# CognitiveAISystems/pogema

Measured on AMD Instinct MI355X. Metric: agent-steps/sec (whole node), 64-agent 64x64 grid, batch=8192 envs, higher is better.
Workload: dtype u32

## Files before the change

include/pogema_amd.h:

```cpp
#ifndef POGEMA_AMD_H
#define POGEMA_AMD_H

#include <stddef.h>
#include <stdint.h>

#ifdef __cplusplus
extern "C" {
#endif

#define PGX_ABI_VERSION 6

#define PGX_OK 0
#define PGX_E_INVALID (-1)
#define PGX_E_HIP (-2)
#define PGX_E_NOMEM (-3)
#define PGX_E_STATE (-4)
#define PGX_E_PLACEMENT (-5)

#define PGX_COLLISION_PRIORITY 0
#define PGX_COLLISION_BLOCK_BOTH 1
#define PGX_COLLISION_SOFT 2

#define PGX_ON_TARGET_FINISH 0
#define PGX_ON_TARGET_RESTART 1
// ... 49 lines not shown
typedef struct pgx_env pgx_env;

int pgx_abi_version(void);
const char* pgx_last_error(void);

int pgx_create(const pgx_config* cfg, int device, pgx_env** out);
int pgx_destroy(pgx_env* env);
int pgx_check_config(const pgx_config* cfg);

int64_t pgx_obs_elems(const pgx_env* env);
int64_t pgx_agent_elems(const pgx_env* env);

int pgx_reset_from_state(pgx_env* env, const uint8_t* obstacles, const int32_t* agent_xy,
                         const int32_t* target_xy, void* stream);

int pgx_reset_random(pgx_env* env, float density, uint64_t seed, const uint8_t* shared_map,
                     const uint8_t* env_mask, int32_t max_retries, void* stream);

int pgx_regenerate(pgx_env* env, const uint8_t* env_mask, float density, uint64_t seed, const uint8_t* shared_map,
                   int32_t max_retries, void* obs, void* stream);
int64_t pgx_regenerate_failures(pgx_env* env, void* stream);

int pgx_set_map_pool(pgx_env* env, const uint8_t* maps, int32_t num_maps, int32_t* capacity_out, void* stream);
int pgx_reset_pool(pgx_env* env, uint64_t seed, const uint8_t* env_mask, int32_t max_retries, void* stream);
int pgx_regenerate_pool(pgx_env* env, const uint8_t* env_mask, uint64_t seed, int32_t max_retries, void* obs,
                        void* stream);
int pgx_get_map_index(pgx_env* env, int32_t* map_index, void* stream);

int pgx_get_map(pgx_env* env, uint8_t* obstacles, void* stream);

int pgx_step(pgx_env* env, const void* actions, int action_dtype, void* obs, float* rewards,
             uint8_t* terminated, uint8_t* truncated, uint8_t* is_active, void* stream);

int pgx_step_held(pgx_env* env, const void* actions, int action_dtype, void* obs, uint8_t* held, int32_t refresh,
                  float* rewards, uint8_t* terminated, uint8_t* truncated, uint8_t* is_active, void* stream);
int pgx_held_available(const pgx_env* env);

int pgx_xcd_shares(pgx_env* env, int32_t* shares);
int pgx_xcd_tune(pgx_env* env, void* obs, void* obs_alt, int32_t rounds, float* us_equal, float* us_tuned, void* stream);

typedef struct pgx_geometry {
    int32_t lanes_per_env;
    int32_t waves;
    int32_t envs_per_wave;
    int32_t multi_wave;
    int32_t p16;
    int32_t stagger;
    int32_t store_policy;
    int32_t state_stores;
    int32_t grid;
    int32_t lds_bytes;
    int32_t for_rollout;
    int32_t xcd_aware;
} pgx_geometry;
int pgx_get_geometry(const pgx_env* env, int32_t for_rollout, pgx_geometry* out);

typedef struct pgx_rollout_io {
    const void* actions;
    void* obs;
    float* rewards;
    uint8_t* terminated;
    uint8_t* truncated;
    uint8_t* is_active;
    uint8_t* episode_done;
    float* metrics;
    int32_t action_dtype;
    int32_t obs_slots;
    int64_t obs_slot_stride;
    uint64_t policy_seed;
// ... 140 lines not shown
```

pogema_amd/_lib.py:

```python
from __future__ import annotations

import ctypes as C
import os

_HERE = os.path.dirname(os.path.abspath(__file__))
LIB_PATH = os.environ.get("PGX_LIB") or os.path.join(_HERE, "libpogema_amd.so")

PGX_ABI_VERSION = 6

COLLISION_SYSTEMS = {"priority": 0, "block_both": 1, "soft": 2}
ON_TARGET = {"finish": 0, "restart": 1, "nothing": 2}
ACTION_DTYPES = {"int8": 0, "int32": 1, "int64": 2}
SOFT_VERTEX_RULES = {"lowest_index": 0, "all_stay": 1}
SOFT_OCCUPANCY = {"index_order": 0, "exact": 1}
COOP_REWARDS = {"all_solved": 0, "per_agent": 1}
BAD_ACTIONS = {"noop": 0, "flag": 1}
LIFELONG_RNGS = {"build": 0, "numpy": 1}
def _obs_dtypes():
    import torch
    return {torch.float32: 0, torch.uint8: 1, torch.bfloat16: 2, torch.float16: 3}


def obs_elem_bytes(dtype) -> int:
    import torch
# ... 9 lines not shown
    def __contains__(self, k):
        self._fill()
        return dict.__contains__(self, k)

    def __getitem__(self, k):
        self._fill()
        return dict.__getitem__(self, k)


OBS_DTYPES = _LazyObsDtypes()
METRIC_NAMES = ("ISR", "CSR", "ep_length", "SoC", "makespan", "avg_throughput")
MAX_OBS_RADIUS, MAX_AGENTS, MAX_SIDE = 15, 1024, 1024
MAX_NEIGHBOURS = 32
DIRECTIONS_FORMATS = {"float32": 0, "uint8": 1, "bits": 2}
SHIELD_TIE_BREAKS = {None: 0, "distance": 1}
MAX_PLAN_HORIZON = 256
PLAN_FIXED_PRIORITY = 1
OUTCOMES = ("STAY", "MOVED", "OBSTACLE", "SWAP", "OCCUPIED", "FOLLOW", "CONTESTED")
NUM_OUTCOMES = len(OUTCOMES)
POLICY_CHANNELS = {"obstacles": 0, "agents": 1, "target": 2, "other_goals": 3, "up": 4, "down": 5, "left": 6, "right": 7}
NUM_CHANNELS = len(POLICY_CHANNELS)
COPY_NO_CACHE = 1
DEFAULT_POLICY_CHANNELS = ("obstacles", "agents", "target", "up", "down", "left", "right")
GLOBAL_CHANNELS = {"obstacles": 0, "agents": 1, "targets": 2, "agent_ids": 3, "target_ids": 4}
NUM_GLOBAL_CHANNELS = len(GLOBAL_CHANNELS)
DEFAULT_GLOBAL_CHANNELS = ("obstacles", "agents", "targets")
GLOBAL_ID_CHANNELS = ("agent_ids", "target_ids")
GLOBAL_ID_MAX = {1: 255, 2: 256}
GLOBAL_BAND_CELLS = 8192


EXPORTED_SYMBOLS = (
    "pgx_abi_version", "pgx_last_error", "pgx_create", "pgx_check_config", "pgx_destroy", "pgx_obs_elems", "pgx_agent_elems",
    "pgx_reset_from_state", "pgx_reset_random", "pgx_regenerate", "pgx_regenerate_failures", "pgx_get_map", "pgx_step", "pgx_step_held", "pgx_held_available", "pgx_observe", "pgx_set_metrics_buffers", "pgx_get_state", "pgx_generate", "pgx_place_agents",
    "pgx_snapshot_bytes", "pgx_save_snapshot", "pgx_load_snapshot", "pgx_time_observe", "pgx_bad_action_count",
    "pgx_buffers_create", "pgx_buffers_ptr", "pgx_buffers_get_info", "pgx_buffers_destroy", "pgx_set_targets",
    "pgx_np_streams", "pgx_np_streams_host", "pgx_np_generate", "pgx_np_generate_host", "pgx_rollout", "pgx_buffers_stride", "pgx_buffers_drop", "pgx_xcd_shares", "pgx_xcd_tune", "pgx_buffers_create_at", "pgx_time_observe_pair", "pgx_buffers_va_reserved", "pgx_get_geometry",
    "pgx_expert_actions", "pgx_set_map_pool", "pgx_reset_pool", "pgx_regenerate_pool", "pgx_get_map_index",
    "pgx_cost_to_go", "pgx_cost_to_go_bytes", "pgx_cost_to_go_builds", "pgx_visible_agents", "pgx_pibt_actions",
    "pgx_goal_directions", "pgx_shield_actions", "pgx_pibt_plan", "pgx_move_outcomes",
    "pgx_policy_input", "pgx_copy_envs", "pgx_global_state", "pgx_global_state_check",
)


class PgxError(RuntimeError):
    def __init__(self, code: int, message: str):
        super().__init__(f"pogema_amd engine error {code}: {message}")
        self.code = code


class PgxBuffersInfo(C.Structure):
    _fields_ = [("bytes", C.c_int64), ("count", C.c_int32), ("spread", C.c_int32), ("candidates", C.c_int32),
                ("reserved0", C.c_int32), ("same_zone_us", C.c_float), ("final_us", C.c_float), ("spacer_gib", C.c_double),
                ("buffer_gbs", C.c_float), ("reserved1", C.c_float)]


class PgxGeometry(C.Structure):
    _fields_ = [(n, C.c_int32) for n in ("lanes_per_env", "waves", "envs_per_wave", "multi_wave", "p16", "stagger",
                                          "store_policy", "state_stores", "grid", "lds_bytes", "for_rollout", "xcd_aware")]


class PgxRolloutIO(C.Structure):
    _fields_ = [("actions", C.c_void_p), ("obs", C.c_void_p), ("rewards", C.c_void_p), ("terminated", C.c_void_p),
                ("truncated", C.c_void_p), ("is_active", C.c_void_p), ("episode_done", C.c_void_p), ("metrics", C.c_void_p),
                ("action_dtype", C.c_int32), ("obs_slots", C.c_int32), ("obs_slot_stride", C.c_int64),
                ("policy_seed", C.c_uint64), ("policy_step0", C.c_int64), ("actions_out", C.c_void_p)]

# ... 96 lines not shown
    lib.pgx_move_outcomes.restype = C.c_int
    lib.pgx_policy_input.argtypes = [vp, C.POINTER(i32), i32, i32, vp, vp]
    lib.pgx_policy_input.restype = C.c_int
    lib.pgx_global_state.argtypes = [vp, C.POINTER(i32), i32, i32, vp, vp]
    lib.pgx_global_state.restype = C.c_int
    lib.pgx_global_state_check.argtypes = [i32, C.POINTER(i32), i32, i32, vp]
    lib.pgx_global_state_check.restype = C.c_int
    lib.pgx_copy_envs.argtypes = [vp, vp, vp, i32, i32, vp]
    lib.pgx_copy_envs.restype = C.c_int
    lib.pgx_set_map_pool.argtypes = [vp, vp, i32, vp, vp]
    lib.pgx_set_map_pool.restype = C.c_int
    lib.pgx_reset_pool.argtypes = [vp, u64, vp, i32, vp]
    lib.pgx_reset_pool.restype = C.c_int
    lib.pgx_regenerate_pool.argtypes = [vp, vp, u64, i32, vp, vp]
    lib.pgx_regenerate_pool.restype = C.c_int
    lib.pgx_get_map_index.argtypes = [vp, vp, vp]
    lib.pgx_get_map_index.restype = C.c_int
    lib.pgx_set_targets.argtypes = [vp, vp, vp, vp]
    lib.pgx_set_targets.restype = C.c_int
    lib.pgx_bad_action_count.argtypes = [vp, vp]
    lib.pgx_bad_action_count.restype = i64
    lib.pgx_time_observe.argtypes = [vp, vp, i32, C.POINTER(C.c_float), vp]
    lib.pgx_time_observe.restype = C.c_int
    lib.pgx_time_observe_pair.argtypes = [vp, vp, vp, i32, C.POINTER(C.c_float), vp]
    lib.pgx_time_observe_pair.restype = C.c_int
    lib.pgx_snapshot_bytes.argtypes = [vp]
    lib.pgx_snapshot_bytes.restype = i64
    lib.pgx_save_snapshot.argtypes = [vp, vp, vp]
    lib.pgx_load_snapshot.argtypes = [vp, vp, vp]
    lib.pgx_save_snapshot.restype = lib.pgx_load_snapshot.restype = C.c_int
    lib.pgx_step.argtypes = [vp, vp, C.c_int, vp, vp, vp, vp, vp, vp]
    lib.pgx_step_held.argtypes = [vp, vp, C.c_int, vp, vp, i32, vp, vp, vp, vp, vp]
    lib.pgx_held_available.argtypes = [vp]
    lib.pgx_step_held.restype = lib.pgx_held_available.restype = C.c_int
    lib.pgx_observe.argtypes = [vp, vp, vp]
    lib.pgx_set_metrics_buffers.argtypes = [vp, vp, vp]
    lib.pgx_get_state.argtypes = [vp, vp, vp, vp, vp, vp, vp]
    lib.pgx_generate.argtypes = [i32, i32, i32, i32, f32, u64, i64, i32, i32, vp, vp, vp]
    lib.pgx_place_agents.argtypes = [i32, i32, i32, i32, u64, i64, i32, i32, vp, i32, vp, vp]
    for name in ("pgx_create", "pgx_destroy", "pgx_reset_from_state", "pgx_reset_random", "pgx_regenerate", "pgx_get_map",
                 "pgx_step", "pgx_observe", "pgx_set_metrics_buffers", "pgx_set_metrics_buffers",
                 "pgx_get_state", "pgx_generate", "pgx_place_agents"):
        getattr(lib, name).restype = C.c_int
    if lib.pgx_abi_version() != PGX_ABI_VERSION:
        raise ImportError(f"{LIB_PATH}: ABI version {lib.pgx_abi_version()} != expected {PGX_ABI_VERSION}; rebuild")
    _lib = lib
    return lib


def check(status: int) -> None:
    if status != 0:
        msg = load().pgx_last_error()
        raise PgxError(status, msg.decode("utf-8", "replace") if msg else "unknown error")
```

pogema_amd/buffers.py:

```python
from __future__ import annotations

import atexit
import collections
import contextlib
import ctypes as C
import os
import threading

import numpy as np
import torch

from . import _lib

_TYPESTR = {torch.float32: "<f4", torch.uint8: "|u1", torch.float16: "<f2", torch.bfloat16: "<f2"}


class _Owner:

    def __init__(self, lib, handle):
        self._lib, self._handle = lib, handle

    def __del__(self):
        try:
            if self._handle is not None and self._handle.value:
# ... 284 lines not shown
            cdata = master.untyped_storage()._cdata
            base = hook(cdata)
            alias = master.detach()
            one = hook(cdata)
            view = alias[2:4].view(torch.int16)
            two = hook(cdata)
            del alias
            still = hook(cdata)
            del view
            back = hook(cdata)
            if not (one == base + 1 and two == base + 2 and still == base + 1 and back == base):
                why = f"torch._C._storage_Use_Count no longer counts tensors per storage ({base}, {one}, {two}, {still}, {back})"
        except Exception as exc:
            why = f"torch._C._storage_Use_Count self-test raised {exc!r}"
    if why is not None:
        import warnings
        warnings.warn(f"pogema_amd: {why} in torch {torch.__version__}; reuse_buffers='recycle' falls back to allocating "
                      f"fresh output tensors per step", RuntimeWarning, stacklevel=2)
        hook = None
    _HOOK = hook
    return hook


_UNSET = object()
_HOOK = _UNSET


class RecyclingOutputs:

    @staticmethod
    def available() -> bool:
        return storage_count_hook() is not None

    def __init__(self, obs_tensors, batch: int, agents: int, zone_ptrs=()):
        if not self.available():
            raise RuntimeError("torch._C._storage_Use_Count is missing or changed its meaning in this torch build")
        self._count = storage_count_hook()
        self._zone_ptrs = frozenset(int(p) for p in zone_ptrs)
        dev = obs_tensors[0].device
        n = batch * agents
        self._sets = []
        for obs in obs_tensors:
            block = torch.empty(n * 7 + 16, dtype=torch.uint8, device=dev)
            members = (obs, block[:4 * n].view(torch.float32).view(batch, agents),
                       block[4 * n:5 * n].view(torch.bool).view(batch, agents),
                       block[5 * n:6 * n].view(torch.bool).view(batch, agents),
                       block[6 * n:7 * n].view(torch.bool).view(batch, agents))
            storages = (obs.untyped_storage(), block.untyped_storage())
            self._sets.append((members, storages, tuple(st._cdata for st in storages)))
        del obs, block, members, storages
        self._idle = [tuple(self._count(c) for c in cdata) for _, _, cdata in self._sets]
        self._held = [torch.full((batch, agents), 255, dtype=torch.uint8, device=dev) for _ in self._sets]
        self._vouched = [None] * len(self._sets)
        self._next = 0
        self.taken = 0
        self.misses = 0

    def __len__(self):
        return len(self._sets)

    def obs_pointers(self):
        return [members[0].data_ptr() for members, _, _ in self._sets]

    def _is_idle(self, i: int) -> bool:
        cdata, idle = self._sets[i][2], self._idle[i]
        return self._count(cdata[0]) == idle[0] and self._count(cdata[1]) == idle[1]

    def free_sets(self) -> int:
        return sum(self._is_idle(i) for i in range(len(self._sets)))

    def retire(self):
        idle = [i for i in range(len(self._sets)) if self._is_idle(i)]
        out = [self._sets[i][0][0] for i in idle if self._sets[i][0][0].data_ptr() in self._zone_ptrs]
        for i in reversed(idle):
            del self._sets[i]
            del self._idle[i]
            del self._held[i]
            del self._vouched[i]
        self._next = 0
        return out

    def _take_index(self):
        n = len(self._sets)
        for k in range(n):
            i = (self._next + k) % n
            if self._is_idle(i):
                self._next = (i + 1) % n
                self.taken += 1
                return i
        self.misses += 1
        return None

    def _hand_out(self, i: int, with_obs: bool):
        m = self._sets[i][0]
        return (m[0].detach() if with_obs else None, m[1].detach(), m[2].detach(), m[3].detach(), m[4].detach())

    @staticmethod
    def _version(t):
        try:
            return t._version
        except Exception:
            return None

    def take(self, with_obs: bool = True):
        i = self._take_index()
        if i is None:
            return None
        if with_obs:
            self._vouched[i] = None
        return self._hand_out(i, with_obs)
# ... 15 lines not shown
```

pogema_amd/csrc/pgx_api.cpp:

```cpp
#include "../../include/pogema_amd.h"

#include <hip/hip_runtime.h>

#include <algorithm>
#include <cstdarg>
#include <cstdio>
#include <cstdlib>
#include <cstring>
#include <new>
#include <string>
#include <vector>

#include "pgx_internal.h"

namespace {
thread_local std::string g_err;
}

namespace pgx {
int fail_msg(int code, const char* fmt, ...) {
    char buf[512];
    va_list ap;
    va_start(ap, fmt);
    vsnprintf(buf, sizeof buf, fmt, ap);
// ... 881 lines not shown
int pgx_get_map(pgx_env* e, uint8_t* obstacles, void* stream) {
    if (!e || !obstacles) return fail_msg(PGX_E_INVALID, "pgx_get_map: null argument");
    DeviceGuard guard;
    if (const int rc = enter(guard, e, "pgx_get_map", true)) return rc;
    PGX_HIP(hipMemcpyAsync(obstacles, e->map_u8, (size_t)e->cfg.batch * e->cfg.height * e->cfg.width,
                           hipMemcpyDeviceToDevice, (hipStream_t)stream));
    return PGX_OK;
}

int pgx_step(pgx_env* e, const void* actions, int action_dtype, void* obs, float* rewards, uint8_t* terminated,
             uint8_t* truncated, uint8_t* is_active, void* stream) {
    if (!e || !actions || !rewards || !terminated || !truncated) return fail_msg(PGX_E_INVALID, "pgx_step: null argument");
    if (const int rc = check_action_dtype("pgx_step", action_dtype)) return rc;
    DeviceGuard guard;
    if (const int rc = enter(guard, e, "pgx_step", true)) return rc;
    pgx::StepParams p = step_params(e, e->geo);
    p.mode = pgx::MODE_STEP;
    p.action_dtype = action_dtype;
    p.actions = actions;
    p.obs = static_cast<float*>(obs);
    p.rewards = rewards;
    p.terminated = terminated;
    p.truncated = truncated;
    p.act_out = is_active;
    PGX_HIP(pgx::launch_step(p, e->geo, (hipStream_t)stream));
    return PGX_OK;
}

int pgx_held_available(const pgx_env* e) {
    if (!e) return 0;
    return pgx::held_available(e->geo, e->cfg.num_agents, e->W, obs_elem_bytes(e->cfg.obs_dtype)) ? 1 : 0;
}

int pgx_step_held(pgx_env* e, const void* actions, int action_dtype, void* obs, uint8_t* held, int32_t refresh, float* rewards,
                  uint8_t* terminated, uint8_t* truncated, uint8_t* is_active, void* stream) {
    if (!e || !obs || !held || !pgx_held_available(e))
        return pgx_step(e, actions, action_dtype, obs, rewards, terminated, truncated, is_active, stream);
    if (!actions || !rewards || !terminated || !truncated) return fail_msg(PGX_E_INVALID, "pgx_step_held: null argument");
    if (const int rc = check_action_dtype("pgx_step_held", action_dtype)) return rc;
    DeviceGuard guard;
    if (const int rc = enter(guard, e, "pgx_step_held", true)) return rc;
    pgx::StepParams p = step_params(e, e->geo);
    p.mode = pgx::MODE_STEP;
    p.action_dtype = action_dtype;
    p.actions = actions;
    p.obs = static_cast<float*>(obs);
    p.rewards = rewards;
    p.terminated = terminated;
    p.truncated = truncated;
    p.act_out = is_active;
    PGX_HIP(pgx::launch_step_held(p, e->geo, held, refresh != 0, (hipStream_t)stream));
    return PGX_OK;
}

int pgx_rollout(pgx_env* e, int32_t steps, const pgx_rollout_io* io, void* stream) {
    if (!e || !io || !io->rewards || !io->terminated || !io->truncated)
        return fail_msg(PGX_E_INVALID, "pgx_rollout: null argument");
    if (io->policy_step0 < 0 || io->policy_step0 > ((int64_t)1 << 40))
        return fail_msg(PGX_E_INVALID, "pgx_rollout: policy_step0 outside 0..2^40");
    if (steps < 1) return fail_msg(PGX_E_INVALID, "pgx_rollout: steps must be >= 1, got %d", steps);
    if (const int rc = check_action_dtype("pgx_rollout", io->action_dtype)) return rc;
    if (io->obs && io->obs_slots < 1) return fail_msg(PGX_E_INVALID, "pgx_rollout: obs given but obs_slots = %d", io->obs_slots);
    DeviceGuard guard;
    if (const int rc = enter(guard, e, "pgx_rollout", true)) return rc;
    pgx::StepParams p = step_params(e, e->geo_roll);
    p.mode = pgx::MODE_STEP;
    p.action_dtype = io->action_dtype;
    p.actions = io->actions;
    p.obs = static_cast<float*>(io->obs);
    p.rewards = io->rewards;
    p.terminated = io->terminated;
    p.truncated = io->truncated;
    p.act_out = io->is_active;
    p.metrics_out = io->metrics;
    p.episode_done = io->episode_done;
    const int64_t agents = (int64_t)e->cfg.batch * e->cfg.num_agents;
    const int64_t W = 2 * e->cfg.obs_radius + 1;
    static const int64_t action_bytes[3] = {1, 4, 8};
    pgx::RolloutParams rp;
    rp.steps = steps;
    rp.obs_slots = io->obs ? io->obs_slots : 1;
    rp.resident_bitmap = e->geo_roll.resident_bitmap ? 1 : 0;
    rp.reserved0 = 0;
    rp.actions_stride = agents * action_bytes[io->action_dtype];
// ... 554 lines not shown
```

pogema_amd/csrc/pgx_internal.h:

```cpp
#pragma once
#include <hip/hip_runtime.h>
#include <stddef.h>
#include <stdint.h>

namespace pgx {

int fail_msg(int code, const char* fmt, ...);

#define PGX_HIP(call)                                                                                                      \
    do {                                                                                                                   \
        const hipError_t e__ = (call);                                                                                     \
        if (e__ != hipSuccess)                                                                                             \
            return pgx::fail_msg(PGX_E_HIP, "%s failed: %s (%s:%d)", #call, hipGetErrorString(e__), __FILE__, __LINE__); \
    } while (0)

struct DeviceGuard {
    int prev = -1;
    bool changed = false;
    hipError_t err = hipSuccess;
    DeviceGuard() = default;
    explicit DeviceGuard(int dev) { (void)select(dev); }
    DeviceGuard(const DeviceGuard&) = delete;
    DeviceGuard& operator=(const DeviceGuard&) = delete;
    hipError_t select(int dev) {
// ... 78 lines not shown
    int32_t xcd_n[8];
    int32_t xcd_base[8];
    uint32_t flags;
    uint64_t seed;
    int64_t env_index_base;
    const uint32_t* obst;
    uint32_t* pos;
    uint32_t* tgt;
    uint8_t* active;
    int32_t* elapsed;
    const uint32_t* pos0;
    const uint32_t* tgt0;
    const uint32_t* comp_begin;
    const uint32_t* comp_len;
    const uint32_t* comp_cells;
    uint32_t* tcount;
    NpGen* np_state;
    const NpGen* np_state0;
    int4* macc;
    float* metrics_out;
    uint8_t* episode_done;
    uint32_t* bad_count;
    const void* actions;
    float* obs;
    float* rewards;
    uint8_t* terminated;
    uint8_t* truncated;
    uint8_t* act_out;
    const uint8_t* only;
    unsigned long long* dbg;
};

struct HeldParams {
    uint8_t* held;
    int32_t refresh;
    int32_t lds_word;
    int32_t words;
};

struct RolloutParams {
    int32_t steps;
    int32_t obs_slots;
    int32_t resident_bitmap;
    int32_t reserved0;
    int64_t actions_stride;
    int64_t agents_stride;
    int64_t envs_stride;
    int64_t obs_stride;
    uint64_t policy_seed;
    int64_t policy_step0;
    int8_t* actions_out;
};

struct StepGeometry {
    int G;
    int waves;
    int epw;
    bool multi_wave;
    bool p16;
    int stagger;
    int store_policy;
    int state_stores;
    bool big;
    bool pc;
    bool resident_bitmap;
    size_t lds_bytes;
    int grid;
    int32_t xcd_n[8], xcd_base[8];
};
StepGeometry step_geometry(int batch, int A, int bmw, int W, bool allow_p16, int epw_override, int obs_elem_bytes,
                           int waves_override, bool for_rollout = false);
hipError_t prepare_step(const StepGeometry& g, const StepGeometry& roll);
hipError_t raise_lds_limit(const void* fn, size_t lds_bytes);
hipError_t launch_step(const StepParams& p, const StepGeometry& g, hipStream_t stream);
bool held_available(const StepGeometry& g, int A, int W, int obs_elem_bytes);
hipError_t prepare_step_held(const StepGeometry& g, int A, int W);
hipError_t launch_step_held(const StepParams& p, const StepGeometry& g, uint8_t* held, bool refresh, hipStream_t stream);
int xcd_partition(int blocks, const float w[8], int32_t n[8], int32_t base[8]);
hipError_t launch_rollout(const StepParams& p, const RolloutParams& rp, const StepGeometry& g, hipStream_t stream);

hipError_t launch_pack_obstacles(const uint8_t* obstacles, const uint8_t* only, uint32_t* bm, int batch, int H, int Wd,
                                 int r, int wpr, int bmw, const OutsideParams& outside, hipStream_t stream);

struct ResetParams {
    int32_t env_begin, env_count;
    int32_t H, Wd, A, r, wpr, bmw;
    int32_t lifelong;
    int32_t given_state;
    int32_t max_retries;
    uint32_t thr;
    uint64_t gen_seed;
    int64_t env_index_base;
    const uint8_t* shared_map;
    uint8_t* todo;
    const uint32_t* epoch;
    uint8_t* scratch_map;
    uint32_t* labels;
    uint32_t* pending;
    uint8_t* map_u8;
    uint32_t* obst_bm;
    uint32_t *pos, *tgt, *pos0, *tgt0;
    uint8_t* active;
    uint32_t* tcount;
    NpGen* np_state;
    const NpGen* np_state0;
    int32_t* elapsed;
    int4* macc;
    uint32_t *comp_begin, *comp_len, *comp_cells;
    uint32_t* fail_count;
    OutsideParams outside;
// ... 175 lines not shown
```

pogema_amd/csrc/pgx_kernels.hip:

```cpp
#include <hip/hip_runtime.h>
#include <stdint.h>
#include <stdlib.h>

#include <array>
#include <type_traits>
#include <map>
#include <mutex>
#include <string>
#include <vector>
#include <utility>

#include "pgx_internal.h"
#include "pgx_nprng.h"

namespace pgx {

__device__ __forceinline__ uint32_t lifelong_draw(uint64_t seed, uint64_t env_index, uint32_t agent,
                                                  uint32_t counter, uint32_t n) {
    uint64_t h = gen_sm64(seed);
    h = gen_sm64(h ^ env_index);
    h = gen_sm64(h ^ (((uint64_t)agent << 32) | counter));
    return (uint32_t)(((h >> 32) * (uint64_t)n) >> 32);
}

// ... 733 lines not shown

        if (p.obs && valid) {
            const int la = MW ? tid : (env_l * A + alane);
            s_apos[la] = pos;
            s_atgt[la] = tgt;
            if (vis != NOCELL_A && !ghost) {
                const uint32_t x = pos >> 16, y = pos & 0xFFFFu;
                atomicOr(&s_occ[env_l * bmw + x * wpr + (y >> 5)], 1u << (y & 31));
            }
        }
    }
    if constexpr (ROLL) {
      if (do_resolve) {
        c.pos = pos;
        c.tgt = tgt;
        c.active = active;
        c.elapsed = so.do_reset ? 0 : elapsed;
        if (fetch_block) {
            uint32_t b = 0u;
#pragma unroll
            for (int k = 0; k < 8; ++k) b |= pack_action4(araw[k]) << (4 * k);
            c.anext = b;
        }
      }
    }
    if (dbg && tid == 0) p.dbg[(size_t)blk * 4 + (dbg2 ? 3 : 1)] = wall_clock64();
    if (!p.obs) {
        if (late_stores) emit_state(pos, tgt, active, elapsed, macc, so);
        return;
    }
    if constexpr (PC) {
        if (!do_stream) return;
    }
    if constexpr (HELD) {
        for (int i = tid; i < hp.words; i += NT) smem[hp.lds_word + i] = 0u;
    }
    lds_sync<MW>();
    if (when_stores == 1) emit_state(pos, tgt, active, elapsed, macc, so);
    int out_slot = slot;
    if constexpr (PC) out_slot = slot == 0 ? rp.obs_slots - 1 : slot - 1;
    float* const obs_out = ROLL ? reinterpret_cast<float*>(reinterpret_cast<char*>(p.obs) + (size_t)out_slot * (size_t)rp.obs_stride) : p.obs;

    if constexpr (P16) {
        const int W_rt = W, r_rt = r;
        uint32_t* rows_base = smem;
        if constexpr (ROLL) rows_base = rp.resident_bitmap ? s_occ : smem;
        if constexpr (PC) rows_base = s_obst + epw * bmw + 2 * (epw * bmw + 2 * AS);
        auto p16_phases = [&](auto wt_tag) {
        constexpr int WT = decltype(wt_tag)::value;
        const int W = WT ? WT : W_rt;
        const int r = WT ? (WT - 1) / 2 : r_rt;
        const uint32_t wmask = (1u << W) - 1u;
        constexpr int RW = WT ? (WT + 1) / 2 : 8;
        [[maybe_unused]] uint32_t held_was = 255u;
        if constexpr (HELD) {
            if (tid < nag && !hp.refresh) held_was = hp.held[(size_t)env0 * A + tid];
        }
        uint32_t rp[3][RW];
#pragma unroll
        for (int t = 0; t < 3; ++t) {
#pragma unroll
            for (int m = 0; m < RW; ++m) rp[t][m] = 0u;
            const int item = tid + t * NT;
            if (item < nag * 3) {
                const int la = item / 3;
                const int c = item - la * 3;
                const int el = MW ? 0 : (p.a_magic ? (int)__umulhi((uint32_t)la, p.a_magic) : la);
                const uint32_t cell = s_apos[la];
                const int x = (int)(cell >> 16), y = (int)(cell & 0xFFFFu);
                if (c < 2) {
                    const uint32_t* bm;
                    if constexpr (BIG) bm = c == 0 ? p.obst + (size_t)env0 * bmw : s_occ;
                    else bm = (c == 0 ? s_obst : s_occ) + el * bmw;
                    const int start = y - r;
                    const int w0 = start >> 5, sh = start & 31;
                    if constexpr (WT == 0) {
#pragma unroll
                        for (int wy = 0; wy < 16; ++wy) {
                            if (wy < W) {
                                const uint32_t* rowp = bm + (x - r + wy) * wpr + w0;
                                const uint32_t bits = (uint32_t)((((uint64_t)rowp[1] << 32) | rowp[0]) >> sh) & wmask;
                                rp[t][wy >> 1] |= bits << (16 * (wy & 1));
                            }
                        }
                    } else {
                    const uint32_t* row0 = bm + (x - r) * wpr + w0;
                        constexpr int RB = WT == 11 ? 6 : WT == 15 ? 5 : 7;
    #pragma unroll
                        for (int w8 = 0; w8 < (WT ? WT : 16); w8 += RB) {
                            uint32_t lo[RB], hi[RB];
    #pragma unroll
                            for (int k = 0; k < RB; ++k) {
                                const int wy = w8 + k;
                                if (wy < (WT ? WT : 16) && (WT || wy < W)) {
                                    lo[k] = row0[wy * wpr];
                                    hi[k] = row0[wy * wpr + 1];
                                }
                            }
    #pragma unroll
                            for (int k = 0; k < RB; ++k) {
                                const int wy = w8 + k;
                                if (wy < (WT ? WT : 16) && (WT || wy < W)) {
                                    const uint32_t bits = (uint32_t)((((uint64_t)hi[k] << 32) | lo[k]) >> sh) & wmask;
                                    rp[t][wy >> 1] |= bits << (16 * (wy & 1));
                                }
                            }
                            asm volatile("" ::: "memory");
                        }
                    }
                } else {
                    const uint32_t tc = s_atgt[la];
                    int dx = x - (int)(tc >> 16), dy = y - (int)(tc & 0xFFFFu);
                    dx = max(-r, min(r, dx));
                    dy = max(-r, min(r, dy));
                    const int hit = r - dx;
                    const uint32_t val = (1u << (r - dy)) << (16 * (hit & 1));
#pragma unroll
                    for (int m = 0; m < RW; ++m) rp[t][m] = (m == (hit >> 1)) ? val : 0u;
                }
            }
        }
        if constexpr (HELD) {
            if (tid < nag) {
                const int la = tid;
                const uint32_t cell = s_apos[la], tc = s_atgt[la];
                const int dx = max(-r, min(r, (int)(cell >> 16) - (int)(tc >> 16)));
                const int dy = max(-r, min(r, (int)(cell & 0xFFFFu) - (int)(tc & 0xFFFFu)));
                const uint32_t now = (uint32_t)((r - dx) * W + (r - dy));
                hp.held[(size_t)env0 * A + la] = (uint8_t)now;
                if (held_was < (uint32_t)(W * W)) {
                    constexpr int UL = PGX_HELD_UNIT_LOG2;
                    const uintptr_t slice = reinterpret_cast<uintptr_t>(obs_out + (size_t)env0 * A * 3 * W * W);
                    const uintptr_t plane = slice + (size_t)(la * 3 + 2) * (size_t)(W * W) * 4;
                    const uintptr_t ub = slice >> UL;
                    const int u1 = (int)(((plane + (size_t)(W * W) * 4) >> UL) - ub);
                    const int uw = (int)(((plane + held_was * 4) >> UL) - ub), un = (int)(((plane + now * 4) >> UL) - ub);
                    for (int u = (int)(((plane + ((1u << UL) - 1u)) >> UL) - ub); u < u1; ++u)
                        if (u != uw && u != un) atomicOr(&smem[hp.lds_word + (u >> 5)], 1u << (u & 31));
                }
            }
        }
        lds_sync<MW>();
        uint16_t* rows16 = reinterpret_cast<uint16_t*>(rows_base);
#pragma unroll
        for (int t = 0; t < 3; ++t) {
            const int item = tid + t * NT;
            if (item < nag * 3) {
#pragma unroll
                for (int wy = 0; wy < (WT ? WT : 16); ++wy)
                    if (WT || wy < W) rows16[item * W + wy] = (uint16_t)(rp[t][wy >> 1] >> (16 * (wy & 1)));
            }
        }
        if (tid < 4) rows16[nag * 3 * W + tid] = 0;
        lds_sync<MW>();

        const int n = nag * 3 * W * W;
        const size_t base = (size_t)env0 * A * 3 * W * W;
        if constexpr (WT == 0) {
        if (p.obs_one && W >= 7) {
            uint16_t* o = reinterpret_cast<uint16_t*>(obs_out) + base;
            const int head = min(n, (int)((8 - (base & 7)) & 7));
            const int nvec = (n - head) >> 3;
            const int tail0 = head + (nvec << 3);
            if (tid < 16) {
                const int e = (tid < 8) ? tid : tail0 + (tid - 8);
                if ((tid < 8) ? (tid < head) : (e < n)) {
                    const int row = (int)__umulhi((uint32_t)e, p.w_magic);
                    o[e] = (uint16_t)((((uint32_t)rows16[row] >> (e - row * W)) & 1u) * p.obs_one);
                }
            }
            const bool span = MW && !(p.flags & 512u);
            const int part = (nvec + nw - 1) / nw;
            const int q0 = span ? wave * part + lane : tid, q1 = span ? min(nvec, (wave + 1) * part) : nvec;
// ... 7 lines not shown
                else if (p.store_policy == 1) stream_rows16_loop_h16<1>(out4, rows32, W, row0, e0 - row0 * W, q0, q1, qs, p.obs_one);
                else stream_rows16_loop_h16<2>(out4, rows32, W, row0, e0 - row0 * W, q0, q1, qs, p.obs_one);
            }
            if (when_stores == 2) emit_state(pos, tgt, active, elapsed, macc, so);
            return;
        }
        if (p.obs_one) {
            const int nrows = nag * 3 * W;
            stream_obs_h16(reinterpret_cast<uint16_t*>(obs_out), base, n, W, p.w_magic, tid, NT, p.store_policy == 1, p.obs_one,
                           [&](int row) -> uint32_t { return row < nrows ? (uint32_t)rows16[row] : 0u; }, wave,
                           (MW && !(p.flags & 512u)) ? nw : 1);
            if (when_stores == 2) emit_state(pos, tgt, active, elapsed, macc, so);
            return;
        }
        if (p.obs_u8) {
            if (dbg && !dbg2 && tid == 0) p.dbg[(size_t)blk * 4 + 2] = wall_clock64();
            const int nrows = nag * 3 * W;
            stream_obs_u8(reinterpret_cast<uint8_t*>(obs_out), base, n, W, p.w_magic, tid, NT, p.store_policy == 1,
                          [&](int row) -> uint32_t { return row < nrows ? (uint32_t)rows16[row] : 0u; }, wave,
                          (MW && !(p.flags & 512u)) ? nw : 1);
            if (when_stores == 2) emit_state(pos, tgt, active, elapsed, macc, so);
            if (dbg && !dbg2 && tid == 0) {
                __builtin_amdgcn_s_waitcnt(0);
                p.dbg[(size_t)blk * 4 + 3] = wall_clock64();
            }
            return;
        }
        }
        float* out = obs_out + base;
        const int head = min(n, (int)((4 - (base & 3)) & 3));
        const uint32_t magic = p.w_magic;
        const int nvec = (n - head) >> 2;
        const int tail0 = head + (nvec << 2);
        stream_rows16_edges(out, rows16, n, head, tail0, W, magic, tid);
        if (dbg && !dbg2 && tid == 0) p.dbg[(size_t)blk * 4 + 2] = wall_clock64();
        const bool span = MW && !(p.flags & 512u);
        const int part = (nvec + nw - 1) / nw;
        const int q0 = span ? wave * part + lane : tid, q1 = span ? min(nvec, (wave + 1) * part) : nvec;
        if constexpr (HELD) {
            const uintptr_t o4 = reinterpret_cast<uintptr_t>(out + head);
            const int a0 = (int)((o4 >> 4) - ((reinterpret_cast<uintptr_t>(out) >> PGX_HELD_UNIT_LOG2) << (PGX_HELD_UNIT_LOG2 - 4)));
            stream_rows16_span<true, true>(reinterpret_cast<f32x4_t*>(out + head), reinterpret_cast<const uint32_t*>(rows16), head, W,
                                           magic, (uint32_t)p.store_policy, q0, q1, span ? 64 : NT, (nag * 3 * W) >> 1,
                                           smem + hp.lds_word, a0, hp.words - 1);
        } else
        stream_rows16_span<true>(reinterpret_cast<f32x4_t*>(out + head), reinterpret_cast<const uint32_t*>(rows16), head, W, magic,
                           (uint32_t)p.store_policy, q0, q1, span ? 64 : NT, (nag * 3 * W) >> 1);
        if (when_stores == 2) emit_state(pos, tgt, active, elapsed, macc, so);
        if (dbg && !dbg2 && tid == 0) {
            __builtin_amdgcn_s_waitcnt(0);
            p.dbg[(size_t)blk * 4 + 3] = wall_clock64();
        }
        return;
        };
        if (p.obs_u8 || p.obs_one) p16_phases(std::integral_constant<int, 0>{});
        else if (W_rt == 11) p16_phases(std::integral_constant<int, 11>{});
        else if (W_rt == 15) p16_phases(std::integral_constant<int, 15>{});
        else if (W_rt == 7) p16_phases(std::integral_constant<int, 7>{});
        else p16_phases(std::integral_constant<int, 0>{});
        return;
    }

    {
        const uint32_t wmask = (W >= 32) ? 0xFFFFFFFFu : ((1u << W) - 1u);
        for (int item = tid; item < nag * 3; item += NT) {
            const int la = item / 3;
// ... 425 lines not shown
    int given = 0, grid = 0;
    for (int x = 0; x < 8; ++x) {
        acc += (double)w[x];
        int upto = x == 7 ? blocks : (int)(acc * blocks + 0.5);
        if (upto > blocks) upto = blocks;
        if (upto < given) upto = given;
        n[x] = upto - given;
        base[x] = given;
        given = upto;
        if (n[x] > grid) grid = n[x];
    }
    return grid * 8;
}

static const void* held_fn_for(const StepGeometry& g) {
    if (g.big || !g.p16) return nullptr;
    if (g.multi_wave) return reinterpret_cast<const void*>(&step_held<64, true>);
#define PGX_CASE(gg) case gg: return reinterpret_cast<const void*>(&step_held<gg, false>);
    switch (g.G) {
        PGX_CASE(1) PGX_CASE(2) PGX_CASE(4) PGX_CASE(8) PGX_CASE(16) PGX_CASE(32) PGX_CASE(64)
        default: return nullptr;
    }
#undef PGX_CASE
}

static int held_words(size_t slice_bytes) {
    const size_t units = (slice_bytes >> PGX_HELD_UNIT_LOG2) + 2;
    return (int)(units / 32 + 1);
}

bool held_available(const StepGeometry& g, int A, int W, int obs_elem_bytes) {
    if (!held_fn_for(g) || obs_elem_bytes != 4 || W > 15) return false;
    const size_t slice = (size_t)g.epw * A * 3 * W * W * 4;
    return g.lds_bytes + (size_t)held_words(slice) * 4 <= 160 * 1024;
}

hipError_t prepare_step_held(const StepGeometry& g, int A, int W) {
    const size_t slice = (size_t)g.epw * A * 3 * W * W * 4;
    return raise_lds_limit(held_fn_for(g), g.lds_bytes + (size_t)held_words(slice) * 4);
}

hipError_t launch_step_held(const StepParams& p, const StepGeometry& g, uint8_t* held, bool refresh, hipStream_t stream) {
    const void* fn = held_fn_for(g);
    if (!fn) return hipErrorInvalidValue;
    StepParams args = p;
    HeldParams h;
    const int W = 2 * p.r + 1;
    h.held = held;
    h.refresh = refresh ? 1 : 0;
    h.lds_word = (int32_t)(g.lds_bytes / 4);
    h.words = held_words((size_t)g.epw * p.num_agents * 3 * W * W * 4);
    void* kargs[] = {&args, &h};
    return hipLaunchKernel(fn, dim3(g.grid), dim3(64 * g.waves), kargs, g.lds_bytes + (size_t)h.words * 4, stream);
}

hipError_t launch_step(const StepParams& p, const StepGeometry& g, hipStream_t stream) {
    const void* fn = step_fn_for(g);
    if (!fn) return hipErrorInvalidValue;
    StepParams args = p;
    void* kargs[] = {&args};
    return hipLaunchKernel(fn, dim3(g.grid), dim3(64 * g.waves), kargs, g.lds_bytes, stream);
}


hipError_t launch_pack_obstacles(const uint8_t* obstacles, const uint8_t* only, uint32_t* bm, int batch, int H, int Wd,
                                 int r, int wpr, int bmw, const OutsideParams& outside, hipStream_t stream) {
    const size_t total = (size_t)batch * bmw;
    const int bs = 256;
    hipLaunchKernelGGL(pack_obstacles_kernel, dim3((unsigned)((total + bs - 1) / bs)), dim3(bs), 0, stream,
                       obstacles, only, bm, batch, H, Wd, r, wpr, bmw, outside);
    return hipGetLastError();
}

hipError_t launch_pack_agents(const int32_t* agent_xy, const int32_t* target_xy, uint32_t* pos, uint32_t* tgt,
                              uint32_t* pos0, uint32_t* tgt0, uint8_t* active, uint32_t* tcount, size_t n,
                              int r, hipStream_t stream, NpGen* np_state, const NpGen* np_state0) {
    const int bs = 256;
    hipLaunchKernelGGL(pack_agents_kernel, dim3((unsigned)((n + bs - 1) / bs)), dim3(bs), 0, stream, agent_xy,
                       target_xy, pos, tgt, pos0, tgt0, active, tcount, n, r, np_state, np_state0);
    return hipGetLastError();
}
// ... 37 lines not shown
```

pogema_amd/placement.py:

```python
from __future__ import annotations

import ctypes as C
import os
from typing import Optional

import numpy as np
import torch

from . import _lib


def choose_buffers(zone_us, plain_us, n, margin=0.98):
    chosen = [("zone", i) for i in range(min(n, len(zone_us)))]
    time_of = {"zone": zone_us, "torch": plain_us}
    for j, t in enumerate(plain_us):
        if len(chosen) < n:
            chosen.append(("torch", j))
            continue
        worst = max(chosen, key=lambda c: time_of[c[0]][c[1]])
        if t < margin * time_of[worst[0]][worst[1]]:
            chosen[chosen.index(worst)] = ("torch", j)
    return chosen


# ... 169 lines not shown
        if probe:
            self.placement.update(probe)
        if fallback is not None:
            self.placement["fallback"] = fallback
            torch.cuda.empty_cache()
        bufs = [torch.empty(self.obs_shape, dtype=self.obs_dtype, device=self.device) for _ in range(n)]
        if self.placement_probe and self.batch >= 2048:
            self.placement.update(self.tune_xcd_shares(bufs[0], bufs[-1] if n > 1 else None))
        return bufs

    @staticmethod
    def _recycle_sets(obs_bytes: int) -> int:
        return 2 if (64 << 20) <= obs_bytes < (256 << 20) else 3

    def _build_recycler(self):
        from .buffers import RecyclingOutputs
        if not RecyclingOutputs.available():
            return False
        obs_bytes = int(np.prod(self.obs_shape)) * _lib.obs_elem_bytes(self.obs_dtype)
        n = self._recycle_sets(obs_bytes)
        if not self.placement_probe or obs_bytes < self.PLACEMENT_MIN_BYTES:
            bufs = self._plain_obs_buffers(n)
        else:
            from .buffers import ParkedBuffers
            parked = ParkedBuffers.claim(self._shelf_key(), n)
            if parked is not None:
                bufs, info = parked
                self._zone_ptrs = {t.data_ptr() for t in bufs}
                self.placement = dict(info, method="pgx_buffers (two HBM zones per buffer; taken over from a closed environment)")
                if self.batch >= 2048:
                    self.placement.update(self.tune_xcd_shares(bufs[0], bufs[-1] if n > 1 else None))
            else:
                bufs = self._pick_obs_buffers(n)
        return RecyclingOutputs(bufs, self.batch, self.num_agents, zone_ptrs=self._zone_ptrs)

    def tune_xcd_shares(self, obs: torch.Tensor, obs_alt: Optional[torch.Tensor] = None, rounds: int = 6) -> dict:
        if not self._has_state():
            return {}
        eq, tuned = C.c_float(0.0), C.c_float(0.0)
        _lib.check(self._lib.pgx_xcd_tune(self._handle, obs.data_ptr(), obs_alt.data_ptr() if obs_alt is not None else None,
                                          int(rounds), C.byref(eq), C.byref(tuned), self._stream()))
        shares = (C.c_int32 * 8)()
        _lib.check(self._lib.pgx_xcd_shares(self._handle, shares))
        return {"xcd_shares": list(shares), "observe_us_equal_shares": round(eq.value, 1), "observe_us_tuned_shares": round(tuned.value, 1)}

    PLAIN_CANDIDATES = 8

    SPARE_BUFFERS = 4

    def _time_observe(self, obs: torch.Tensor, obs_alt: Optional[torch.Tensor] = None) -> float:
        if not self._has_state():
            return 0.0
        us = C.c_float(0.0)
        if obs_alt is not None:
            _lib.check(self._lib.pgx_time_observe_pair(self._handle, obs.data_ptr(), obs_alt.data_ptr(), 8, C.byref(us), self._stream()))
            return float(us.value)
        _lib.check(self._lib.pgx_time_observe(self._handle, obs.data_ptr(), 3, C.byref(us), self._stream()))
        return float(us.value)

    def _ring_from_recycler(self, slots: int, obs_bytes: int):
        if not self.recycle or self._recycler is False:
            return None
        if self._recycler is None:
            if not self._has_state() or torch.cuda.is_current_stream_capturing():
                return None
            self._recycler = self._build_recycler()
        rec = self._recycler
# ... 90 lines not shown
```

pogema_amd/vec_env.py:

```python
from __future__ import annotations

import ctypes as C
import os
import warnings
from typing import Optional

import numpy as np
import torch

from . import _lib
from .grid_config import GridConfig
from .placement import PlacementMixin, choose_buffers
from .queries import QueryMixin
from .semantics import Semantics


def _as_device_index(device) -> int:
    dev = torch.device(device)
    if dev.type != "cuda":
        raise ValueError(f"VecPogema runs on a HIP device only, got {device!r}")
    return dev.index if dev.index is not None else torch.cuda.current_device()


def parse_map_pool(maps) -> torch.Tensor:
# ... 559 lines not shown
        if actions.device != self.device:
            actions = actions.to(self.device, non_blocking=True)
        if actions.dtype not in (torch.int8, torch.int32, torch.int64):
            actions = actions.to(torch.int64)
        if actions.numel() != self.batch * self.num_agents:
            raise ValueError(f"expected {self.batch}x{self.num_agents} actions, got shape {tuple(actions.shape)}")
        return actions.contiguous()

    _ACTION_CODE = {torch.int8: 0, torch.int32: 1, torch.int64: 2}

    def _check_out(self, out):
        if len(out) != 5:
            raise ValueError("out must be (obs, rewards, terminated, truncated, is_active)")
        B, A = self.batch, self.num_agents
        want = ((self.obs_shape, self.obs_dtype), ((B, A), torch.float32), ((B, A), torch.bool), ((B, A), torch.bool),
                ((B, A), torch.bool))
        for name, t, (shape, dtype) in zip(("obs", "rewards", "terminated", "truncated", "is_active"), out, want):
            if t is None and name == "obs":
                continue
            ok_dtype = t.dtype == dtype or (dtype == torch.bool and t.dtype == torch.uint8)
            if tuple(t.shape) != tuple(shape) or not ok_dtype or not t.is_contiguous() or t.device != self.device:
                raise ValueError(f"out[{name}] must be a contiguous {dtype} tensor of shape {tuple(shape)} on {self.device}")
        return out

    def step(self, actions, compute_obs: bool = True, out=None):
        actions = self._prepare_actions(actions)
        if out is not None:
            obs, rewards, terminated, truncated, is_active = self._check_out(out)
            if compute_obs and obs is None:
                raise ValueError("out[obs] is None but compute_obs=True")
        else:
            held = self._held_outputs(compute_obs) if self._held_on else None
            if held is not None:
                (obs, rewards, terminated, truncated, is_active), record, trusted, index = held
                if compute_obs:
                    _lib.check(self._lib.pgx_step_held(
                        self._handle, actions.data_ptr(), self._ACTION_CODE[actions.dtype], obs.data_ptr(), record.data_ptr(),
                        0 if trusted else 1, rewards.data_ptr(), terminated.data_ptr(), truncated.data_ptr(),
                        is_active.data_ptr(), self._stream()))
                    self._recycler.vouch(index)
                    self._held_steps += 1
                    self._held_refreshes += 0 if trusted else 1
                    infos = {"is_active": is_active, "episode_done": self.episode_done, "metrics": self.metrics}
                    if self.semantics.bad_action == "flag":
                        self._raise_on_bad_actions()
                    return self._wrap_obs(obs), rewards, terminated, truncated, infos
            elif self._held_on and self._recycler and not torch.cuda.is_current_stream_capturing():
                obs, rewards, terminated, truncated, is_active = self._alloc_outputs(compute_obs)
            else:
                obs, rewards, terminated, truncated, is_active = self._outputs(compute_obs)
        _lib.check(self._lib.pgx_step(
            self._handle, actions.data_ptr(), self._ACTION_CODE[actions.dtype],
            obs.data_ptr() if compute_obs else None, rewards.data_ptr(), terminated.data_ptr(),
            truncated.data_ptr(), is_active.data_ptr(), self._stream()))
        if self.regenerate:
            if self._reset_seed is None:
                raise RuntimeError("auto_reset='regenerate' needs reset(seed) first (random instances)")
            if self._pool is not None:
                _lib.check(self._lib.pgx_regenerate_pool(
                    self._handle, self.episode_done.data_ptr(), self._reset_seed, 3,
                    obs.data_ptr() if compute_obs else None, self._stream()))
            else:
                if self._shared is None and self.grid_config.map is not None:
                    self._shared = self._shared_map_tensor()
                _lib.check(self._lib.pgx_regenerate(
                    self._handle, self.episode_done.data_ptr(), float(self.grid_config.density), self._reset_seed,
                    self._shared.data_ptr() if self._shared is not None else None, 3,
                    obs.data_ptr() if compute_obs else None, self._stream()))
        if self.semantics.bad_action == "flag":
            self._raise_on_bad_actions()
# ... 159 lines not shown
```

Measured before the change: 5.265 billion.

## Track zero obs store units per buffer via ballot bitmask instead of per-agent held cell

Replaces the per-agent 'held target cell' record with a per-block bitmask of obs store units that were all-zero when last written into a recycled output buffer. The kernel computes each unit's zero verdict with a wave ballot, records it for the buffer, and combines it with the previous record to skip rewriting units that are still zero. This generalizes skipping beyond the target plane so more redundant global stores can be avoided. In exchange it adds per-unit zero checks from LDS rows, extra global mask traffic per step, and a tighter availability condition on mask size.

```diff
diff --git a/include/pogema_amd.h b/include/pogema_amd.h
--- a/include/pogema_amd.h
+++ b/include/pogema_amd.h
@@ -105,9 +105,12 @@
 int pgx_step(pgx_env* env, const void* actions, int action_dtype, void* obs, float* rewards,
              uint8_t* terminated, uint8_t* truncated, uint8_t* is_active, void* stream);
 
+int pgx_step_held_lines(pgx_env* env, const void* actions, int action_dtype, void* obs, uint32_t* lines, int32_t refresh,
+                        float* rewards, uint8_t* terminated, uint8_t* truncated, uint8_t* is_active, void* stream);
+int64_t pgx_held_lines_words(const pgx_env* env);
+int pgx_held_available(const pgx_env* env);
 int pgx_step_held(pgx_env* env, const void* actions, int action_dtype, void* obs, uint8_t* held, int32_t refresh,
                   float* rewards, uint8_t* terminated, uint8_t* truncated, uint8_t* is_active, void* stream);
-int pgx_held_available(const pgx_env* env);
 
 int pgx_xcd_shares(pgx_env* env, int32_t* shares);
 int pgx_xcd_tune(pgx_env* env, void* obs, void* obs_alt, int32_t rounds, float* us_equal, float* us_tuned, void* stream);
diff --git a/pogema_amd/_lib.py b/pogema_amd/_lib.py
--- a/pogema_amd/_lib.py
+++ b/pogema_amd/_lib.py
@@ -65,7 +65,7 @@
 
 EXPORTED_SYMBOLS = (
     "pgx_abi_version", "pgx_last_error", "pgx_create", "pgx_check_config", "pgx_destroy", "pgx_obs_elems", "pgx_agent_elems",
-    "pgx_reset_from_state", "pgx_reset_random", "pgx_regenerate", "pgx_regenerate_failures", "pgx_get_map", "pgx_step", "pgx_step_held", "pgx_held_available", "pgx_observe", "pgx_set_metrics_buffers", "pgx_get_state", "pgx_generate", "pgx_place_agents",
+    "pgx_reset_from_state", "pgx_reset_random", "pgx_regenerate", "pgx_regenerate_failures", "pgx_get_map", "pgx_step", "pgx_step_held", "pgx_step_held_lines", "pgx_held_lines_words", "pgx_held_available", "pgx_observe", "pgx_set_metrics_buffers", "pgx_get_state", "pgx_generate", "pgx_place_agents",
     "pgx_snapshot_bytes", "pgx_save_snapshot", "pgx_load_snapshot", "pgx_time_observe", "pgx_bad_action_count",
     "pgx_buffers_create", "pgx_buffers_ptr", "pgx_buffers_get_info", "pgx_buffers_destroy", "pgx_set_targets",
     "pgx_np_streams", "pgx_np_streams_host", "pgx_np_generate", "pgx_np_generate_host", "pgx_rollout", "pgx_buffers_stride", "pgx_buffers_drop", "pgx_xcd_shares", "pgx_xcd_tune", "pgx_buffers_create_at", "pgx_time_observe_pair", "pgx_buffers_va_reserved", "pgx_get_geometry",
@@ -228,7 +228,10 @@
     lib.pgx_step.argtypes = [vp, vp, C.c_int, vp, vp, vp, vp, vp, vp]
     lib.pgx_step_held.argtypes = [vp, vp, C.c_int, vp, vp, i32, vp, vp, vp, vp, vp]
     lib.pgx_held_available.argtypes = [vp]
-    lib.pgx_step_held.restype = lib.pgx_held_available.restype = C.c_int
+    lib.pgx_step_held_lines.argtypes = [vp, vp, C.c_int, vp, vp, i32, vp, vp, vp, vp, vp]
+    lib.pgx_held_lines_words.argtypes = [vp]
+    lib.pgx_step_held.restype = lib.pgx_step_held_lines.restype = lib.pgx_held_available.restype = C.c_int
+    lib.pgx_held_lines_words.restype = C.c_int64
     lib.pgx_observe.argtypes = [vp, vp, vp]
     lib.pgx_set_metrics_buffers.argtypes = [vp, vp, vp]
     lib.pgx_get_state.argtypes = [vp, vp, vp, vp, vp, vp, vp]
diff --git a/pogema_amd/buffers.py b/pogema_amd/buffers.py
--- a/pogema_amd/buffers.py
+++ b/pogema_amd/buffers.py
@@ -340,7 +340,7 @@
     def available() -> bool:
         return storage_count_hook() is not None
 
-    def __init__(self, obs_tensors, batch: int, agents: int, zone_ptrs=()):
+    def __init__(self, obs_tensors, batch: int, agents: int, zone_ptrs=(), line_words: int = 0):
         if not self.available():
             raise RuntimeError("torch._C._storage_Use_Count is missing or changed its meaning in this torch build")
         self._count = storage_count_hook()
@@ -359,6 +359,7 @@
         del obs, block, members, storages
         self._idle = [tuple(self._count(c) for c in cdata) for _, _, cdata in self._sets]
         self._held = [torch.full((batch, agents), 255, dtype=torch.uint8, device=dev) for _ in self._sets]
+        self._lines = [torch.zeros(int(line_words), dtype=torch.int32, device=dev) for _ in self._sets]
         self._vouched = [None] * len(self._sets)
         self._next = 0
         self.taken = 0
@@ -366,6 +367,9 @@
 
     def __len__(self):
         return len(self._sets)
+
+    def lines(self, i: int):
+        return self._lines[i]
 
     def obs_pointers(self):
         return [members[0].data_ptr() for members, _, _ in self._sets]
@@ -384,6 +388,7 @@
             del self._sets[i]
             del self._idle[i]
             del self._held[i]
+            del self._lines[i]
             del self._vouched[i]
         self._next = 0
         return out
diff --git a/pogema_amd/csrc/pgx_api.cpp b/pogema_amd/csrc/pgx_api.cpp
--- a/pogema_amd/csrc/pgx_api.cpp
+++ b/pogema_amd/csrc/pgx_api.cpp
@@ -937,14 +937,26 @@
     return pgx::held_available(e->geo, e->cfg.num_agents, e->W, obs_elem_bytes(e->cfg.obs_dtype)) ? 1 : 0;
 }
 
+int64_t pgx_held_lines_words(const pgx_env* e) {
+    if (!pgx_held_available(e)) return 0;
+    return (int64_t)pgx::held_record_words(e->geo, e->cfg.batch, e->cfg.num_agents, e->W);
+}
+
 int pgx_step_held(pgx_env* e, const void* actions, int action_dtype, void* obs, uint8_t* held, int32_t refresh, float* rewards,
                   uint8_t* terminated, uint8_t* truncated, uint8_t* is_active, void* stream) {
-    if (!e || !obs || !held || !pgx_held_available(e))
+    (void)held;
+    (void)refresh;
+    return pgx_step(e, actions, action_dtype, obs, rewards, terminated, truncated, is_active, stream);
+}
+
+int pgx_step_held_lines(pgx_env* e, const void* actions, int action_dtype, void* obs, uint32_t* lines, int32_t refresh,
+                        float* rewards, uint8_t* terminated, uint8_t* truncated, uint8_t* is_active, void* stream) {
+    if (!e || !obs || !lines || !pgx_held_available(e))
         return pgx_step(e, actions, action_dtype, obs, rewards, terminated, truncated, is_active, stream);
-    if (!actions || !rewards || !terminated || !truncated) return fail_msg(PGX_E_INVALID, "pgx_step_held: null argument");
-    if (const int rc = check_action_dtype("pgx_step_held", action_dtype)) return rc;
-    DeviceGuard guard;
-    if (const int rc = enter(guard, e, "pgx_step_held", true)) return rc;
+    if (!actions || !rewards || !terminated || !truncated) return fail_msg(PGX_E_INVALID, "pgx_step_held_lines: null argument");
+    if (const int rc = check_action_dtype("pgx_step_held_lines", action_dtype)) return rc;
+    DeviceGuard guard;
+    if (const int rc = enter(guard, e, "pgx_step_held_lines", true)) return rc;
     pgx::StepParams p = step_params(e, e->geo);
     p.mode = pgx::MODE_STEP;
     p.action_dtype = action_dtype;
@@ -954,7 +966,7 @@
     p.terminated = terminated;
     p.truncated = truncated;
     p.act_out = is_active;
-    PGX_HIP(pgx::launch_step_held(p, e->geo, held, refresh != 0, (hipStream_t)stream));
+    PGX_HIP(pgx::launch_step_held(p, e->geo, lines, refresh != 0, (hipStream_t)stream));
     return PGX_OK;
 }
 
diff --git a/pogema_amd/csrc/pgx_internal.h b/pogema_amd/csrc/pgx_internal.h
--- a/pogema_amd/csrc/pgx_internal.h
+++ b/pogema_amd/csrc/pgx_internal.h
@@ -134,7 +134,7 @@
 };
 
 struct HeldParams {
-    uint8_t* held;
+    uint32_t* lines;
     int32_t refresh;
     int32_t lds_word;
     int32_t words;
@@ -177,7 +177,8 @@
 hipError_t launch_step(const StepParams& p, const StepGeometry& g, hipStream_t stream);
 bool held_available(const StepGeometry& g, int A, int W, int obs_elem_bytes);
 hipError_t prepare_step_held(const StepGeometry& g, int A, int W);
-hipError_t launch_step_held(const StepParams& p, const StepGeometry& g, uint8_t* held, bool refresh, hipStream_t stream);
+size_t held_record_words(const StepGeometry& g, int batch, int A, int W);
+hipError_t launch_step_held(const StepParams& p, const StepGeometry& g, uint32_t* lines, bool refresh, hipStream_t stream);
 int xcd_partition(int blocks, const float w[8], int32_t n[8], int32_t base[8]);
 hipError_t launch_rollout(const StepParams& p, const RolloutParams& rp, const StepGeometry& g, hipStream_t stream);
 
diff --git a/pogema_amd/csrc/pgx_kernels.hip b/pogema_amd/csrc/pgx_kernels.hip
--- a/pogema_amd/csrc/pgx_kernels.hip
+++ b/pogema_amd/csrc/pgx_kernels.hip
@@ -789,9 +789,6 @@
     if constexpr (PC) {
         if (!do_stream) return;
     }
-    if constexpr (HELD) {
-        for (int i = tid; i < hp.words; i += NT) smem[hp.lds_word + i] = 0u;
-    }
     lds_sync<MW>();
     if (when_stores == 1) emit_state(pos, tgt, active, elapsed, macc, so);
     int out_slot = slot;
@@ -809,9 +806,9 @@
         const int r = WT ? (WT - 1) / 2 : r_rt;
         const uint32_t wmask = (1u << W) - 1u;
         constexpr int RW = WT ? (WT + 1) / 2 : 8;
-        [[maybe_unused]] uint32_t held_was = 255u;
+        [[maybe_unused]] uint32_t lines_were = 0u;
         if constexpr (HELD) {
-            if (tid < nag && !hp.refresh) held_was = hp.held[(size_t)env0 * A + tid];
+            if (tid < hp.words && !hp.refresh) lines_were = hp.lines[(size_t)blk * hp.words + tid];
         }
         uint32_t rp[3][RW];
 #pragma unroll
@@ -878,24 +875,7 @@
             }
         }
         if constexpr (HELD) {
-            if (tid < nag) {
-                const int la = tid;
-                const uint32_t cell = s_apos[la], tc = s_atgt[la];
-                const int dx = max(-r, min(r, (int)(cell >> 16) - (int)(tc >> 16)));
-                const int dy = max(-r, min(r, (int)(cell & 0xFFFFu) - (int)(tc & 0xFFFFu)));
-                const uint32_t now = (uint32_t)((r - dx) * W + (r - dy));
-                hp.held[(size_t)env0 * A + la] = (uint8_t)now;
-                if (held_was < (uint32_t)(W * W)) {
-                    constexpr int UL = PGX_HELD_UNIT_LOG2;
-                    const uintptr_t slice = reinterpret_cast<uintptr_t>(obs_out + (size_t)env0 * A * 3 * W * W);
-                    const uintptr_t plane = slice + (size_t)(la * 3 + 2) * (size_t)(W * W) * 4;
-                    const uintptr_t ub = slice >> UL;
-                    const int u1 = (int)(((plane + (size_t)(W * W) * 4) >> UL) - ub);
-                    const int uw = (int)(((plane + held_was * 4) >> UL) - ub), un = (int)(((plane + now * 4) >> UL) - ub);
-                    for (int u = (int)(((plane + ((1u << UL) - 1u)) >> UL) - ub); u < u1; ++u)
-                        if (u != uw && u != un) atomicOr(&smem[hp.lds_word + (u >> 5)], 1u << (u & 31));
-                }
-            }
+            if (tid < hp.words) smem[hp.lds_word + tid] = lines_were;
         }
         lds_sync<MW>();
         uint16_t* rows16 = reinterpret_cast<uint16_t*>(rows_base);
@@ -969,6 +949,58 @@
         const uint32_t magic = p.w_magic;
         const int nvec = (n - head) >> 2;
         const int tail0 = head + (nvec << 2);
+        if constexpr (HELD) {
+            uint32_t* skip = smem + hp.lds_word;
+            const int lead = (int)((reinterpret_cast<uintptr_t>(out) & ((1u << PGX_HELD_UNIT_LOG2) - 1u)) >> 2);
+            for (int w = 2 * wave; w < hp.words; w += 2 * nw) {
+                const int e = (w * 32 + lane) * (1 << (PGX_HELD_UNIT_LOG2 - 2)) - lead;
+                bool zero = e >= 0 && e + (1 << (PGX_HELD_UNIT_LOG2 - 2)) <= n;
+                if constexpr (WT != 0) {
+                    constexpr int LF = 1 << (PGX_HELD_UNIT_LOG2 - 2);
+                    constexpr int NR = (LF + 2 * (WT - 1)) / WT, ND = NR / 2 + 1;
+                    const int ec = zero ? e : 0;
+                    const int row = (int)__umulhi((uint32_t)ec, magic);
+                    const int col = ec - row * WT;
+                    const uint32_t* rw = reinterpret_cast<const uint32_t*>(rows16) + (row >> 1);
+                    uint32_t d[ND + 1];
+#pragma unroll
+                    for (int k = 0; k < ND; ++k) d[k] = rw[k];
+                    d[ND] = 0u;
+                    const int par = row & 1;
+                    uint32_t any = 0u;
+#pragma unroll
+                    for (int k = 0; k < NR; ++k) {
+                        const uint32_t lo = d[k >> 1], hi = d[(k >> 1) + 1];
+                        const uint32_t pairw = (k & 1) ? (par ? hi : lo >> 16) : (par ? lo >> 16 : lo);
+                        const uint32_t bits = pairw & 0xFFFFu;
+                        if (k == 0) any = bits >> col;
+                        else {
+                            const int take = max(0, min(WT, LF - (WT - col) - (k - 1) * WT));
+                            any |= bits & ((1u << take) - 1u);
+                        }
+                    }
+                    zero = zero && any == 0u;
+                } else if (zero) {
+                    int row = (int)__umulhi((uint32_t)e, magic);
+                    const int col = e - row * W;
+                    uint32_t any = (uint32_t)rows16[row] >> col;
+                    int left = (1 << (PGX_HELD_UNIT_LOG2 - 2)) - (W - col);
+                    for (; left > 0; left -= W) {
+                        const uint32_t bits = rows16[++row];
+                        any |= left >= W ? bits : (bits & ((1u << left) - 1u));
+                    }
+                    zero = any == 0u;
+                }
+                const uint64_t verdicts = __ballot(zero);
+                const int mine = w + (lane >> 5);
+                if ((lane & 31) == 0 && mine < hp.words) {
+                    const uint32_t now = (uint32_t)(verdicts >> (lane & 32));
+                    skip[mine] &= now;
+                    hp.lines[(size_t)blk * hp.words + mine] = now;
+                }
+            }
+            lds_sync<MW>();
+        }
         stream_rows16_edges(out, rows16, n, head, tail0, W, magic, tid);
         if (dbg && !dbg2 && tid == 0) p.dbg[(size_t)blk * 4 + 2] = wall_clock64();
         const bool span = MW && !(p.flags & 512u);
@@ -1460,7 +1492,13 @@
 bool held_available(const StepGeometry& g, int A, int W, int obs_elem_bytes) {
     if (!held_fn_for(g) || obs_elem_bytes != 4 || W > 15) return false;
     const size_t slice = (size_t)g.epw * A * 3 * W * W * 4;
+    if (held_words(slice) > 64 * g.waves) return false;
     return g.lds_bytes + (size_t)held_words(slice) * 4 <= 160 * 1024;
+}
+
+size_t held_record_words(const StepGeometry& g, int batch, int A, int W) {
+    const size_t slices = g.multi_wave ? (size_t)batch : ((size_t)batch + g.epw - 1) / g.epw;
+    return slices * (size_t)held_words((size_t)g.epw * A * 3 * W * W * 4);
 }
 
 hipError_t prepare_step_held(const StepGeometry& g, int A, int W) {
@@ -1468,13 +1506,13 @@
     return raise_lds_limit(held_fn_for(g), g.lds_bytes + (size_t)held_words(slice) * 4);
 }
 
-hipError_t launch_step_held(const StepParams& p, const StepGeometry& g, uint8_t* held, bool refresh, hipStream_t stream) {
+hipError_t launch_step_held(const StepParams& p, const StepGeometry& g, uint32_t* lines, bool refresh, hipStream_t stream) {
     const void* fn = held_fn_for(g);
     if (!fn) return hipErrorInvalidValue;
     StepParams args = p;
     HeldParams h;
     const int W = 2 * p.r + 1;
-    h.held = held;
+    h.lines = lines;
     h.refresh = refresh ? 1 : 0;
     h.lds_word = (int32_t)(g.lds_bytes / 4);
     h.words = held_words((size_t)g.epw * p.num_agents * 3 * W * W * 4);
diff --git a/pogema_amd/placement.py b/pogema_amd/placement.py
--- a/pogema_amd/placement.py
+++ b/pogema_amd/placement.py
@@ -225,7 +225,8 @@
                     self.placement.update(self.tune_xcd_shares(bufs[0], bufs[-1] if n > 1 else None))
             else:
                 bufs = self._pick_obs_buffers(n)
-        return RecyclingOutputs(bufs, self.batch, self.num_agents, zone_ptrs=self._zone_ptrs)
+        words = int(self._lib.pgx_held_lines_words(self._handle)) if getattr(self, "_held_on", False) else 0
+        return RecyclingOutputs(bufs, self.batch, self.num_agents, zone_ptrs=self._zone_ptrs, line_words=words)
 
     def tune_xcd_shares(self, obs: torch.Tensor, obs_alt: Optional[torch.Tensor] = None, rounds: int = 6) -> dict:
         if not self._has_state():
diff --git a/pogema_amd/vec_env.py b/pogema_amd/vec_env.py
--- a/pogema_amd/vec_env.py
+++ b/pogema_amd/vec_env.py
@@ -615,10 +615,11 @@
         else:
             held = self._held_outputs(compute_obs) if self._held_on else None
             if held is not None:
-                (obs, rewards, terminated, truncated, is_active), record, trusted, index = held
+                (obs, rewards, terminated, truncated, is_active), _, trusted, index = held
                 if compute_obs:
-                    _lib.check(self._lib.pgx_step_held(
-                        self._handle, actions.data_ptr(), self._ACTION_CODE[actions.dtype], obs.data_ptr(), record.data_ptr(),
+                    _lib.check(self._lib.pgx_step_held_lines(
+                        self._handle, actions.data_ptr(), self._ACTION_CODE[actions.dtype], obs.data_ptr(),
+                        self._recycler.lines(index).data_ptr(),
                         0 if trusted else 1, rewards.data_ptr(), terminated.data_ptr(), truncated.data_ptr(),
                         is_active.data_ptr(), self._stream()))
                     self._recycler.vouch(index)
```

After: 5.073 billion. 3.7% lower.
